# abhisrkckl/PulsePortraiture

Hardware: AMD Instinct MI355X
Metric: subint portrait fits/sec (phase+DM, 512ch×2048bin) at 1/2/4/8 MI355X (higher is better)
Workload: dtype f64

## Files before the change

pulseportraiture_amd/csrc/ppf_api.cpp:

```cpp
#include <hip/hip_runtime.h>

#include <algorithm>
#include <atomic>
#include <chrono>
#include <cmath>
#include <cstdarg>
#include <cstdio>
#include <cstdlib>
#include <cstring>
#include <map>
#include <mutex>
#include <string>
#include <thread>
#include <utility>
#include <vector>

#include "../../include/ppfit.h"
#include "ppf_internal.hpp"
#include "ppf_device.hpp"

struct ppf_ctx {
    int device;
    std::string err;
    mutable std::mutex err_mu;
// ... 337 lines not shown
    if (!d) return fail(ctx, PPF_EINVAL, "null descriptor");
    if (d->nsub < 1 || d->nchan < 1) return fail(ctx, PPF_EINVAL, "nsub=%d nchan=%d", d->nsub, d->nchan);
    if (!nbin_supported(d->nbin) && !long_fit_ok(d))
        return fail(ctx, PPF_EUNSUP,
                    "nbin=%d: must be even in [32, 8192] or odd in [33, 4095], or longer without the "
                    "GetTOAs guess (up to 2^23 transform points)", d->nbin);
    if (d->data_dtype != PPF_F32 && d->data_dtype != PPF_F64)
        return fail(ctx, PPF_EINVAL, "data_dtype=%d", d->data_dtype);
    if (d->nmodel < 1) return fail(ctx, PPF_EINVAL, "nmodel=%d", d->nmodel);
    if (!d->data || !d->model || !d->freqs || !d->P || !d->init || !d->fit_flags || !d->nu_fits ||
        !d->nu_outs || !d->results || !d->scales || !d->scale_errs || !d->channel_snrs ||
        !d->covariance)
        return fail(ctx, PPF_EINVAL, "required pointer is NULL");
    if (d->mode != PPF_MODE_FULL && d->mode != PPF_MODE_LEGACY2)
        return fail(ctx, PPF_EINVAL, "mode=%d", d->mode);
    if (d->guess) {
        if (!d->guess_weights || !d->guess_DM) return fail(ctx, PPF_EINVAL, "guess needs weights and DM");
        if (d->guess_Ns < 1 || d->guess_Ns > 65536) return fail(ctx, PPF_EINVAL, "guess_Ns=%d", d->guess_Ns);
    }
    if (!d->workspace) return fail(ctx, PPF_EINVAL, "workspace is NULL");
    FitLayout L = fit_layout(d);
    if (d->workspace_bytes < L.total)
        return fail(ctx, PPF_ENOMEM, "workspace %zu < %zu bytes", d->workspace_bytes, L.total);
    return PPF_OK;
}

using EvPair = std::pair<hipEvent_t, hipEvent_t>;

EvPair *event_pair(std::vector<EvPair> &v, int i, hipError_t *e) {
    if ((int)v.size() <= i) {
        EvPair pr{};
        if ((*e = hipEventCreate(&pr.first)) != hipSuccess) return nullptr;
        if ((*e = hipEventCreate(&pr.second)) != hipSuccess) {
            (void)hipEventDestroy(pr.first);
            return nullptr;
        }
        v.push_back(pr);
    }
    return &v[i];
}

int event_ms(ppf_ctx *ctx, hipEvent_t a, hipEvent_t b, double *ms) {
    hipError_t e = hipEventSynchronize(b);
    if (e != hipSuccess) return hip_fail(ctx, e, "hipEventSynchronize");
    float t = 0.f;
    if ((e = hipEventElapsedTime(&t, a, b)) != hipSuccess) return hip_fail(ctx, e, "hipEventElapsedTime");
    *ms = (double)t;
    return PPF_OK;
}

template <class F>
int for_history(ppf_ctx *ctx, int n, const double *ms, F &&entry) {
    if (!ctx || !ms || n < 0) return PPF_EINVAL;
    if (!ctx->prof) return fail(ctx, PPF_EINVAL, "profiling is off");
    const long avail = ctx->ncalls < ppf_ctx::kRing ? ctx->ncalls : ppf_ctx::kRing;
    if (n > avail) n = (int)avail;
    for (int c = 0; c < n; ++c)
        if (int rc = entry(c, (int)((ctx->ncalls - n + c) % ppf_ctx::kRing))) return rc;
    return n;
}

struct FitCall {
    ppf_ctx *ctx;
    const ppf_fit_desc *d;
    hipStream_t st;
    FitLayout L;
    char *ws;
    const double2 *T, *T2;
    double2 *Mft;
    double *Mpow;
    int nharm, kc;
    int slot;
    bool fused;
    bool bounded;
    uint8_t *needx;
    int32_t *xslot;
    uint8_t *xtile;
    uint8_t *gflag;
    double2 *gpart;
    double *gwx;
    unsigned *kinds;
    int32_t *cls;
    double *rec;

    template <class U>
    U *at(size_t off) const { return (U *)(ws + off); }
    const int32_t *KC() const { return at<const int32_t>(L.KC); }
    unsigned *counts() const { return kinds + 4; }
    void mark(int i) const { if (ctx->prof) (void)hipEventRecord(ctx->ring[slot][i], st); }
    EvPair *solv_begin(int kind) const {
        hipError_t e;
        EvPair *pe = ctx->prof ? event_pair(ctx->solv_ev[slot], ctx->nsolv[slot], &e) : nullptr;
        if (!pe) return nullptr;
        ctx->solv_kind[slot].resize(ctx->solv_ev[slot].size());
        ctx->solv_kind[slot][ctx->nsolv[slot]++] = kind;
        (void)hipEventRecord(pe->first, st);
        return pe;
    }
    void solv_end(EvPair *pe) const { if (pe) (void)hipEventRecord(pe->second, st); }

    int begin();
    int models(), spectra(), guess();
    ppf::SolveArgs solve_args() const;
    ppf::XmomArgs xmom_args(const ppf::SolveArgs &sa) const;
    int round(const ppf::SolveArgs &sa, const ppf::XmomArgs &ma, bool any_pass, bool any_mom, bool first);
    int solve(const ppf::SolveArgs &sa), postfit(const ppf::SolveArgs &sa);
};

int FitCall::begin() {
    hipError_t e = hipSetDevice(ctx->device);
    if (e != hipSuccess) return hip_fail(ctx, e, "hipSetDevice");
    L = fit_layout(d);
    int rc;
    if (!L.lng && (rc = twiddles(ctx, d->nbin, st, &T, &T2))) return rc;
    ws = (char *)d->workspace;
    Mft = at<double2>(L.M); Mpow = at<double>(L.Mpow);
    nharm = d->nbin / 2 + 1; kc = noise_kc(nharm, 4);
    fused = L.fused && !L.momx;
    bounded = (d->options & PPF_OPT_NO_X) != 0;
    needx = at<uint8_t>(L.needx); xslot = at<int32_t>(L.xslot);
    xtile = L.tiled ? at<uint8_t>(L.xtile) : nullptr;
    if (d->guess && L.fused && ppf::xspec_guess_fused_n(rfft_log2(d->nbin))) {
        gflag = at<uint8_t>(L.gflag); gpart = at<double2>(L.gpart); gwx = at<double>(L.gwx);
    }
    kinds = at<unsigned>(L.active + 16); cls = at<int32_t>(L.cls); rec = at<double>(L.rec);
    slot = (int)(ctx->ncalls % ppf_ctx::kRing);
    for (int i = 0; i < 4; ++i) ctx->ran[slot][i] = true;
    ctx->npass[slot] = ctx->nsolv[slot] = 0;
    ctx->ran[slot][2] = d->guess != 0;
    ctx->ran[slot][4] = ctx->ran[slot][5] = false;
    return PPF_OK;
}

int FitCall::models() {
    hipError_t e;
    if (L.lng) {
        if (int rc = long_rfft_rows(ctx, L.lw, ws, d->nbin, (int64_t)d->nmodel * d->nchan, PPF_F64, d->model, Mft,
                                    false, st))
            return rc;
    } else {
        ppf::RfftArgs ra{d->nbin, rfft_log2(d->nbin), PPF_F64, d->model, T, T2, Mft};
        if ((e = ppf::launch_rfft_rows(ra, (int64_t)d->nmodel * d->nchan, st)) != hipSuccess)
            return hip_fail(ctx, e, "k_rfft_rows");
    }
    if ((e = ppf::launch_model_pow_t(Mft, d->nchan, nharm, d->nmodel, at<double>(L.MP), st)) != hipSuccess)
        return hip_fail(ctx, e, "k_model_pow_t");
    if ((e = ppf::launch_model_cut(at<const double>(L.MP), d->nchan, nharm, d->nmodel,
                                   (d->options & PPF_OPT_NO_HCUT) != 0, at<int32_t>(L.KC), st)) != hipSuccess)
        return hip_fail(ctx, e, "k_model_cut");
    if ((e = ppf::launch_model_pow(Mft, d->nchan, nharm, d->nmodel, Mpow, st)) != hipSuccess)
        return hip_fail(ctx, e, "k_model_pow");
    if ((e = hipMemsetAsync(kinds, 0, 8 * sizeof(unsigned), st)) != hipSuccess)
        return hip_fail(ctx, e, "hipMemsetAsync");
    ppf::ClassifyArgs ca{};
    ca.nsub = d->nsub; ca.nchan = d->nchan; ca.log10_tau = d->log10_tau;
    ca.fused = fused ? 1 : 0; ca.xcap = L.xcap;
    ca.fit_flags = d->fit_flags; ca.init = d->init; ca.freqs = d->freqs; ca.P = d->P;
    ca.nu_fits = d->nu_fits; ca.mask = d->chan_mask; ca.model_index = d->model_index;
    ca.KC = KC(); ca.klim = gflag ? 64 * ppf::guess_npl(rfft_log2(d->nbin)) : -1;
    ca.guess_DM = d->guess ? d->guess_DM : nullptr; ca.guess_ref = d->guess ? d->guess_ref : 0;
    ca.needx = needx; ca.xslot = xslot; ca.xtile = xtile; ca.gflag = gflag; ca.cls = cls; ca.rec = rec;
    ca.hm_list = at<int32_t>(L.hmlist); ca.ng_list = at<int32_t>(L.nglist); ca.counts = counts();
    if ((e = ppf::launch_classify(ca, st)) != hipSuccess) return hip_fail(ctx, e, "k_classify");
    return PPF_OK;
}

// ... 124 lines not shown
    if (mr.cb > 8) {
        mr.cb = 8;
        mr.nblk = (mr.nchan + 7) / 8;
        mr.xcd_swizzle = (mr.nblk % 8 == 0) ? 1 : 0;
    }
    return mr;
}

int FitCall::round(const ppf::SolveArgs &sa, const ppf::XmomArgs &ma, bool any_pass, bool any_mom, bool first) {
    hipError_t e;
    if (any_pass) {
        EvPair *pe = nullptr;
        if (ctx->prof) {
            if (!(pe = event_pair(ctx->pass_ev[slot], ctx->npass[slot], &e)))
                return hip_fail(ctx, e, "hipEventCreate");
            ++ctx->npass[slot];
            (void)hipEventRecord(pe->first, st);
        }
        if ((e = ppf::launch_pass(sa, st)) != hipSuccess) return hip_fail(ctx, e, "k_pass");
        if (pe) (void)hipEventRecord(pe->second, st);
    }
    if (any_mom) {
        if (first) mark(5);
        if (!fused) e = ppf::launch_moments(sa, st);
        else e = first ? ppf::launch_xmom(ma, true, st) : ppf::launch_xmom(recentre_args(ma), false, st);
        if (e != hipSuccess) return hip_fail(ctx, e, fused ? "k_xmom" : "k_moments");
        if (first) {
            mark(6);
            ctx->ran[slot][4] = true;
        }
    }
    if ((e = hipMemsetAsync(sa.active, 0, 2 * sizeof(unsigned), st)) != hipSuccess)
        return hip_fail(ctx, e, "hipMemsetAsync");
    if (any_pass) {
        EvPair *pe = solv_begin(1);
        if ((e = ppf::launch_tr_step(sa, st)) != hipSuccess) return hip_fail(ctx, e, "k_tr_step");
        solv_end(pe);
    }
    if (any_mom) {
        EvPair *pe = solv_begin(0);
        if ((e = ppf::launch_tr_mom(sa, st)) != hipSuccess) return hip_fail(ctx, e, "k_tr_mom");
        solv_end(pe);
    }
    return PPF_OK;
}

int FitCall::solve(const ppf::SolveArgs &sa) {
    hipError_t e;
    int rc;
    if (!ctx->host_active && (e = hipHostMalloc((void **)&ctx->host_active, 4 * sizeof(unsigned))) != hipSuccess)
        return hip_fail(ctx, e, "hipHostMalloc");
    if ((e = ppf::launch_tr_init(sa, st)) != hipSuccess) return hip_fail(ctx, e, "k_tr_init");
    const bool spin = (d->options & PPF_OPT_SPIN_WAIT) != 0;
    const bool no_stream = L.fused && L.xcap == 0;
    bool kinds_late = !no_stream && bounded;
    bool any_mom = true, any_pass = false;
    if (!no_stream && !kinds_late) {
        if ((rc = read_back(ctx, ctx->host_active + 1, sa.kinds, 2, st, spin))) return rc;
        any_mom = ctx->host_active[1] != 0;
        any_pass = ctx->host_active[2] != 0;
    }
    const ppf::XmomArgs ma = xmom_args(sa);
    if (fused && (e = ppf::launch_btab(d->nbin / 2, at<double>(L.Bt), st)) != hipSuccess)
        return hip_fail(ctx, e, "k_btab");
    const int maxiter = d->max_iter > 0 ? d->max_iter : 200 * 5;
    int iter = 0;
    for (int group = any_pass ? 3 : 1; any_mom || any_pass; group = 2) {
        for (int g = 0; g < group; ++g)
            if ((rc = round(sa, ma, any_pass, any_mom, iter == 0 && g == 0))) return rc;
        iter += group;
        if (kinds_late && (e = hipMemcpyAsync(ctx->host_active + 1, sa.kinds, 2 * sizeof(unsigned),
                                              hipMemcpyDeviceToHost, st)) != hipSuccess)
            return hip_fail(ctx, e, "hipMemcpyAsync");
        if ((rc = read_back(ctx, ctx->host_active, sa.active, 1, st, spin))) return rc;
        if (kinds_late) {
            kinds_late = false;
            if (ctx->host_active[2] != 0) {
                any_pass = true;
                continue;
            }
        }
        if (*ctx->host_active == 0 || iter > maxiter + 2) break;
    }
    return PPF_OK;
}

int FitCall::postfit(const ppf::SolveArgs &sa) {
    EvPair *pe = solv_begin(2);
    const hipError_t e = ppf::launch_postfit(sa, st);
    if (e != hipSuccess) return hip_fail(ctx, e, "k_postfit");
    solv_end(pe);
    return PPF_OK;
}

}

extern "C" {

int ppf_abi_version(void) { return PPF_ABI_VERSION; }
size_t ppf_sizeof_fit_desc(void) { return sizeof(ppf_fit_desc); }
size_t ppf_sizeof_result(void) { return sizeof(ppf_result); }

int ppf_create(int device, ppf_ctx **out) {
    if (!out) return PPF_EINVAL;
    *out = nullptr;
    int n = 0;
    hipError_t e = hipGetDeviceCount(&n);
    if (e != hipSuccess || n == 0) return PPF_EHIP;
    if (device < 0 || device >= n) return PPF_EINVAL;
    ppf_ctx *c = new ppf_ctx();
    c->device = device;
    *out = c;
    return PPF_OK;
}

void ppf_destroy(ppf_ctx *ctx) {
    if (!ctx) return;
    (void)hipSetDevice(ctx->device);
    for (auto &kv : ctx->tw) (void)hipFree(kv.second);
    for (auto &kv : ctx->cz) (void)hipFree(kv.second);
    for (auto &set : ctx->ring)
        for (auto &e : set)
            if (e) (void)hipEventDestroy(e);
    for (auto &v : ctx->pass_ev)
        for (auto &pr : v) {
            (void)hipEventDestroy(pr.first);
            (void)hipEventDestroy(pr.second);
        }
    for (auto &v : ctx->solv_ev)
        for (auto &pr : v) {
            (void)hipEventDestroy(pr.first);
            (void)hipEventDestroy(pr.second);
        }
    if (ctx->host_active) (void)hipHostFree(ctx->host_active);
    if (ctx->lscr) (void)hipFree(ctx->lscr);
    delete ctx;
}

int ppf_set_profiling(ppf_ctx *ctx, int enable) {
    if (!ctx) return PPF_EINVAL;
    hipError_t e = hipSetDevice(ctx->device);
    if (e != hipSuccess) return hip_fail(ctx, e, "hipSetDevice");
    if (enable && !ctx->ring[0][0])
        for (auto &set : ctx->ring)
            for (auto &ev : set)
                if ((e = hipEventCreate(&ev)) != hipSuccess) return hip_fail(ctx, e, "hipEventCreate");
    ctx->prof = enable != 0;
    ctx->ncalls = 0;
    return PPF_OK;
}

int ppf_stage_ms_history(ppf_ctx *ctx, int n, double *ms) {
    return for_history(ctx, n, ms, [&](int c, int slot) -> int {
        for (int i = 0; i < 4; ++i) {
            ms[c * 4 + i] = 0.0;
            if (!ctx->ran[slot][i]) continue;
            if (int rc = event_ms(ctx, ctx->ring[slot][i], ctx->ring[slot][i + 1], &ms[c * 4 + i])) return rc;
        }
        return PPF_OK;
    });
}

int ppf_kernel_ms_history(ppf_ctx *ctx, int n, double *ms) {
    return for_history(ctx, n, ms, [&](int c, int slot) -> int {
        for (int i = 0; i < 2; ++i) {
            ms[c * 2 + i] = 0.0;
            if (!ctx->ran[slot][4 + i]) continue;
            if (int rc = event_ms(ctx, ctx->ring[slot][5 + 2 * i], ctx->ring[slot][6 + 2 * i], &ms[c * 2 + i]))
                return rc;
        }
        return PPF_OK;
    });
// ... 1251 lines not shown
```

pulseportraiture_amd/csrc/ppf_internal.hpp:

```cpp
#pragma once
#include <hip/hip_runtime.h>
#include <stdint.h>

#include "../../include/ppfit.h"

namespace ppf {

struct RfftArgs {
    int nbin, log2N, dtype;
    const void *in;
    const double2 *T, *T2;
    double2 *out;
};

struct XspecArgs {
    int nsub, nchan, nbin, log2N, kc, nblk, cb, dtype, xcd_swizzle;
    const void *data;
    const double2 *Mft;
    const int32_t *model_index;
    const uint8_t *mask;
    const double *errs;
    const double *freqs, *P;
    const double2 *T, *T2;
    double2 *X;
// ... 42 lines not shown
    const void *data;
    const double2 *Mft;
    const int32_t *model_index;
    const uint8_t *mask;
    double *chan;
    const double *dphi;
    const double2 *T, *T2;
    const void *state;
    double *mom;
    const double *Bt;
    int kc;
    const double *errs;
    const double *Mpow;
    double *mres;
    const int32_t *KC;
    const unsigned *rc_count;
    const int32_t *rc_list;
};

struct GuessArgs {
    int nsub, nchan, nbin, log2N, kc, nblkd, Ns;
    int guess_ref;
    const uint8_t *mask;
    const double *freqs, *P, *guess_DM, *guess_tau, *nu_fits;
    const double *gP;
    const double *gw;
    const double2 *T, *T2;
    double *x0;
    const double2 *Msum;
    const double2 *Mft;
    const int32_t *model_index;
    const int32_t *KC;
    const uint8_t *gflag;
    const double2 *gpart;
    const double *gwx;
    int nblk;
    const double2 *czB, *czT;
    int czP, czJ, czQ, czK;
    const double2 *gspec;
    double *gsh;
};

struct CzPlan {
    int Ns, K, P, J, Q;
};
hipError_t launch_cz_table(const CzPlan &c, double2 *B, const double2 *T, hipStream_t st);

struct TRState;

struct SolveArgs {
    int nsub, nchan, nbin;
    const double2 *X, *Mft;
    const double *MP;
    const int32_t *KC;
    const int32_t *model_index;
    const double *chan;
    const double *freqs, *P;
    const uint8_t *mask;
    const double *init;
    const int32_t *fit_flags;
    const double *nu_fits, *nu_outs;
    const double *bounds;
    int log10_tau, option, is_toa, mode, max_iter, guess;
    int newton;
    const double *x0;
    double *stats;
    ppf_result *results;
    double *scales, *scale_errs, *channel_snrs, *covariance;
    TRState *state;
    double *partials;
    unsigned *active;
    unsigned *kinds;
    double2 *mom;
    double *dphi;
    double *mres;
    int mom16;
    double *hcen;
    const int32_t *xslot;
    const uint8_t *xtile;
    int xnh;
    unsigned *rc_count;
    int32_t *rc_list;
    const double *rec;
};

struct RotateArgs {
    int nbin, log2N, dtype;
    const void *in;
    const double *phases;
    const double2 *T, *T2;
    double *out;
    int ref_len;
    const double2 *Te, *T2e;
};

struct InstRespArgs {
    int nbin;
    const double *src;
    const int32_t *src_row;
    const double *table;
    const double *widths;
    const double2 *T, *T2;
    double *out;
};

struct AlignArgs {
    int nsub, nchan, nbin, log2N, dtype, ngroup;
    const void *in;
    const double *phases;
    const double *weights;
    const double2 *T, *T2;
    double2 *part;
    double *wpart;
    double *out;
    double *wsum;
};
int align_groups(int nsub, int nchan);
hipError_t launch_align(const AlignArgs &a, hipStream_t st);
bool align_wave_supported(int log2N);
hipError_t launch_align_part_w(const AlignArgs &a, hipStream_t st);
hipError_t launch_align_phases(int nsub, int nchan, const double *results, const double *freqs, const double *P,
                               const uint8_t *mask, const double *scales, const double *errs, double *phases,
                               double *weights, hipStream_t st);

struct ResidArgs {
    int nbin, log2N, dtype;
    const void *in;
    const double *phases;
    const double *model;
    const int32_t *model_row;
    const double *scales, *errs;
    double dof;
    const double2 *T, *T2;
    double *out;
};
hipError_t launch_resid_chi2(const ResidArgs &a, int64_t nrows, hipStream_t st);

struct NoiseArgs {
    int nbin, log2N, dtype, kc;
    const void *in;
    const double2 *T, *T2;
    double *out;
};

constexpr int kNfGrid = 20;
struct NoiseFitArgs {
    int nbin, dtype;
    const void *in;
    const double2 *T, *T2;
    int64_t nharm;
    const double *pows;
    const double *errs;
    int64_t errs_len;
    int fn;
    double fact;
    double a_grid[kNfGrid];
    int32_t kc_table[kNfGrid];
    double *noise_out;
    int32_t *kc_out;
    int64_t row0;
};

struct LongNoiseArgs {
    int64_t nbin;
    int64_t n;
    int64_t M, M1, M2;
    int log2M, log2M1;
// ... 303 lines not shown
```

pulseportraiture_amd/csrc/ppf_solve.hip:

```cpp
#include <type_traits>
#include "ppf_device.hpp"
#include "ppf_internal.hpp"
#include "ppf_state.hpp"

namespace ppf {

struct Fac {
    double dphi[3];
    double t[2];
    double u[3];
    bool br_tt, br_ta, br_aa;
};

__device__ __forceinline__ void chan_derivs(const double *st, const Fac &fc, double dC[5],
                                            double dS[5], double d2C[5][5], double d2S[5][5]) {
    const double Cp = st[1], Cpp = st[2], Q1 = st[3], Q1p = st[4], Q2 = st[5];
    const double S1 = st[7], S2a = st[8], S2b = st[9];
    for (int i = 0; i < 3; ++i) { dC[i] = Cp * fc.dphi[i]; dS[i] = 0.0; }
    for (int j = 0; j < 2; ++j) { dC[3 + j] = Q1 * fc.t[j]; dS[3 + j] = S1 * fc.t[j]; }
    for (int i = 0; i < 3; ++i) {
        for (int j = 0; j < 3; ++j) { d2C[i][j] = Cpp * fc.dphi[i] * fc.dphi[j]; d2S[i][j] = 0.0; }
        for (int j = 0; j < 2; ++j) {
            d2C[i][3 + j] = d2C[3 + j][i] = fc.dphi[i] * fc.t[j] * Q1p;
            d2S[i][3 + j] = d2S[3 + j][i] = 0.0;
// ... 1232 lines not shown
                double co[7] = {A * C - E * G, 0.0, E * H - A * D, 0.0, F * G - B * C, 0.0,
                                B * D - F * H};
                double roots[8];
                int nr = poly_real_roots(co, 6, roots);
                double best = 0.0, bd = 1e300;
                bool any = false;
                for (int i = 0; i < nr; ++i)
                    if (roots[i] > 0.0 && fabs(nu_mean - roots[i]) < bd) {
                        bd = fabs(nu_mean - roots[i]); best = roots[i]; any = true;
                    }
                if (any) { nz[0] = nz[1] = best; } else no_root = true;
            }
            break;
        }
        case 0x1b: {
            double T[4][4];
            int q = 12;
            for (int i = 0; i < 4; ++i)
                for (int j = i; j < 4; ++j) { T[i][j] = T[j][i] = c[q]; ++q; }
            double H11 = T[0][0], H22 = T[1][1], H33 = T[2][2], H44 = T[3][3];
            double H12 = T[0][1], H13 = T[0][2], H14 = T[0][3], H23 = T[1][2],
                   H34 = T[2][3];
            num = (H34 * H34 - H33 * H44) * c[0] + (H13 * H44 - H14 * H34) * c[1] +
                  (H14 * H33 - H13 * H34) * c[2];
            den = (H34 * H34 - H33 * H44) * c[3] + (H13 * H44 - H14 * H34) * c[4] +
                  (H14 * H33 - H13 * H34) * c[5];
            nz[0] = pow(num / den, -0.5);
            num = (H13 * H22 - H12 * H23) * c[6] + (H11 * H23 - H12 * H13) * c[7] +
                  (H12 * H12 - H11 * H22) * c[8];
            den = (H13 * H22 - H12 * H23) * c[9] + (H11 * H23 - H12 * H13) * c[10] +
                  (H12 * H12 - H11 * H22) * c[11];
            nz[2] = exp(num / den);
            break;
        }
        case 0xf: {
            if (option == 0 || option == 1) {
                double H14 = c[16], H44 = c[17];
                double A = c[0], aa = c[1], B = c[2], b = c[3], C = c[4], cc = c[5],
                       D = c[6], d = c[7], E = c[8], e = c[9], F = c[10], f = c[11];
                double co[6];
                int deg;
                if (option == 0) {
                    co[0] = A * A * B + H44 * C * D + H14 * E * F - H44 * B * E - A * C * F -
                            H14 * A * D;
                    co[1] = -A * A * b - H44 * C * d - H14 * E * f + H44 * b * E + A * C * f +
                            H14 * A * d;
                    co[2] = -2 * A * aa * B - H44 * cc * D - H14 * e * F + H44 * B * e +
                            (A * cc + aa * C) * F + H14 * aa * D;
                    co[3] = 2 * A * aa * b + H44 * cc * d + H14 * e * f - H44 * b * e -
                            (A * cc + aa * C) * f - H14 * aa * d;
                    co[4] = aa * aa * B - aa * cc * F;
                    co[5] = -aa * aa * b + aa * cc * f;
                    deg = 5;
                } else {
                    co[0] = A * A * B + H44 * C * D + H14 * E * F - H44 * B * E - A * C * F -
                            H14 * A * D;
                    co[1] = -2 * A * aa * B - H44 * cc * D - H14 * e * F + H44 * B * e +
                            (A * cc + aa * C) * F + H14 * aa * D;
                    co[2] = -(A * A * b - aa * aa * B) - H44 * C * d - H14 * E * f +
                            H44 * b * E + (A * C * f - aa * cc * F) + H14 * A * d;
                    co[3] = 2 * A * aa * b + H44 * cc * d + H14 * e * f - H44 * b * e -
                            (A * cc + aa * C) * f - H14 * aa * d;
                    co[4] = -aa * aa * b + aa * cc * f;
                    deg = 4;
                }
                double roots[8];
                int nr = poly_real_roots(co, deg, roots);
                double best = 0.0, bd = 1e300;
                bool any = false;
                for (int i = 0; i < nr; ++i)
                    if (roots[i] > 0.0) {
                        double rr = sqrt(roots[i]);
                        if (fabs(nu_mean - rr) < bd) { bd = fabs(nu_mean - rr); best = rr; any = true; }
                    }
                if (any) { nz[0] = nz[1] = best; } else no_root = true;
            }
            break;
        }
        default: break;
    }
    *no_root_out = no_root ? 1 : 0;
}

template <int PB>
__global__ __launch_bounds__(PB) void k_postfit(SolveArgs a) {
    __shared__ double red[kWaves * 32];
    __shared__ double sh_Xinv[25];
    __shared__ double sh_misc[16];
    __shared__ double sh_acc[NZ_MAX + 8];
    const int s = blockIdx.x, tid = threadIdx.x;
    const TRState &S = a.state[s];
    ppf_result *res = a.results + s;
    if (S.status == PPF_ST_NOFIT || S.status == PPF_ST_NOSPACE) {
        if (tid == 0) {
            for (int i = 0; i < 32; ++i) reinterpret_cast<double *>(res)[i] = 0.0;
            res->status = S.status;
            const double pg = S.phi_guess;
            res->phi_guess = fabs(pg) <= kDblMax ? pg : a.init[(int64_t)s * 5];
        }
        for (int n = tid; n < a.nchan; n += PB) {
            const int64_t o2 = (int64_t)s * a.nchan + n;
            a.scales[o2] = 0.0; a.scale_errs[o2] = 0.0; a.channel_snrs[o2] = 0.0;
        }
        return;
    }
    struct { const double *fr; const uint8_t *mask; int nchan; } v;
    v.fr = a.freqs + (int64_t)s * a.nchan;
    v.mask = a.mask ? a.mask + (int64_t)s * a.nchan : nullptr;
    v.nchan = a.nchan;
    const int flagmask = S.flagmask;
    int idx[5], nf = 0;
    for (int i = 0; i < 5; ++i)
        if (flagmask >> i & 1) idx[nf++] = i;
    double x[5];
    for (int i = 0; i < 5; ++i) x[i] = S.x[i];
    const double fun = S.f;
    const int status = S.status, nfev = S.nfev, k = S.k;
    const bool scat = S.scat != 0;
    const double nu_mean = S.nu_mean, dof = S.dof, phi_guess = S.phi_guess;
    double sdv[1] = {0.0};
    {
        const double *chan = a.chan + (int64_t)s * a.nchan * 4;
        const uint8_t *mk = a.mask ? a.mask + (int64_t)s * a.nchan : nullptr;
        for (int n = tid; n < a.nchan; n += PB)
            if (!mk || mk[n]) sdv[0] += chan[n * 4 + 2];
    }
    blk_sum<1, PB>(sdv, red);
    const double Sd = sdv[0];
    const int nchanx = S.nchanx;
    FitGeom g;
    g.P = a.P[s];
    g.nu_DM = S.nu_fit[0];
    g.nu_GM = S.nu_fit[1];
    g.nu_tau = S.nu_fit[2];
    g.log10_tau = a.log10_tau;
    g.tau_lin = 0.0;
    g.g_sum = g.g_tau = g.g_alpha = false;
    const double *st_fit = a.stats + ((int64_t)s * 2 + S.slot_cur) * a.nchan * 10;

    const double tau_fit_lin = a.log10_tau ? pow(10.0, x[3]) : x[3];
    auto gates = [&](FitGeom &gg, double taulin, double alpha) {
        gg.tau_lin = taulin;
        if (!scat) { gg.g_sum = gg.g_tau = gg.g_alpha = false; return; }
        double sm[3] = {0.0, 0.0, 0.0};
        for (int n = tid; n < v.nchan; n += PB) {
            if (v.mask && !v.mask[n]) continue;
            double tn = taulin * pow(v.fr[n] / gg.nu_tau, alpha);
            sm[0] += tn;
            sm[1] += gg.log10_tau ? kLn10 * tn : tn / taulin;
            sm[2] += log(v.fr[n] / gg.nu_tau) * tn;
        }
        blk_sum<3, PB>(sm, red);
        gg.g_sum = sm[0] != 0.0;
        gg.g_tau = gg.g_sum && sm[1] != 0.0;
        gg.g_alpha = sm[2] != 0.0;
    };
    gates(g, tau_fit_lin, x[4]);

    double nu_out[3];
    bool need_nz = false;
    for (int i = 0; i < 3; ++i) {
        nu_out[i] = a.nu_outs[(int64_t)s * 3 + i];
        if (!(nu_out[i] == nu_out[i]) || nu_out[i] == 0.0) need_nz = true;
    }
    int nzcase = flagmask;
    if (a.mode == PPF_MODE_LEGACY2) nzcase = 0x3;
    if (nzcase == 0x1f) nzcase = 0x1b;
    double nz[3] = {g.nu_DM, g.nu_GM, g.nu_tau};
    bool no_root = false;
    const bool closed = (nzcase == 0x3 || nzcase == 0x5 || nzcase == 0x18 || nzcase == 0xb ||
                         nzcase == 0x7 || nzcase == 0x1b || nzcase == 0xf);
    if (need_nz && closed) {
        double accv[NZ_MAX + 8];
        for (int i = 0; i < NZ_MAX + 8; ++i) accv[i] = 0.0;
        const double cD = kDconst / g.P, cG = kDconst * kDconst / g.P;
        for (int n = tid; n < v.nchan; n += PB) {
            if (v.mask && !v.mask[n]) continue;
            const double *st = st_fit + (int64_t)n * 10;
            const double nu = v.fr[n];
            Fac fc = make_fac(nu, g, x[4]);
            double H[5][5], Hd[5][5], Hg[5][5], Ha[5][5];
            chan_hess(st, fc, H);
            Fac f1 = fc; f1.dphi[1] = 1.0; chan_hess(st, f1, Hd);
            Fac f2 = fc; f2.dphi[2] = 1.0; chan_hess(st, f2, Hg);
            double rd[5], rg[5], ra[5];
            for (int b = 0; b < 5; ++b) { rd[b] = Hd[1][b]; rg[b] = Hg[2][b]; }
            rd[1] = Hd[1][1] * fc.dphi[1];
            rg[2] = Hg[2][2] * fc.dphi[2];
            if (nzcase == 0x18 || nzcase == 0x1b) {
                Fac f3 = fc;
                if (fc.t[1] != 0.0) {
                    f3.u[1] = fc.u[1] / fc.t[1];
                    f3.u[2] = fc.u[2] / fc.t[1];
                }
                f3.t[1] = 1.0;
                chan_hess(st, f3, Ha);
                for (int b = 0; b < 5; ++b) ra[b] = Ha[4][b];
            }
            const double w2 = pow(nu, -2.0), w4 = pow(nu, -4.0), wl = log(nu);
            double *c = accv;
            switch (nzcase) {
                case 0x3: c[0] += w2 * rd[0]; c[1] += rd[0]; break;
                case 0x5: c[0] += w4 * rg[0]; c[1] += rg[0]; break;
                case 0x18: c[0] += wl * ra[3]; c[1] += ra[3]; break;
                case 0xb:
                    c[0] += w2 * rd[3]; c[1] += w2 * rd[0]; c[2] += rd[3]; c[3] += rd[0];
                    c[16] += H[3][0]; c[17] += H[3][3];
                    break;
                case 0x7:
                    if (a.option == 0) {
                        c[0] += w4 * rg[0]; c[1] += rg[0]; c[2] += w2 * rd[2]; c[3] += rd[2];
                        c[4] += w4 * rg[2]; c[5] += rg[2]; c[6] += w2 * rd[0]; c[7] += rd[0];
                    } else {
                        c[0] += w4 * rd[0]; c[1] += rd[0]; c[2] += w2 * rg[1]; c[3] += rg[1];
                        c[4] += w4 * rd[1]; c[5] += rd[1]; c[6] += w2 * rg[0]; c[7] += rg[0];
                    }
                    break;
                case 0x1b:
                    c[0] += w2 * rd[0]; c[1] += w2 * rd[3]; c[2] += w2 * rd[4];
                    c[3] += rd[0]; c[4] += rd[3]; c[5] += rd[4];
                    c[6] += wl * ra[0]; c[7] += wl * ra[1]; c[8] += wl * ra[3];
                    c[9] += ra[0]; c[10] += ra[1]; c[11] += ra[3];
                    {
                        const int r4[4] = {0, 1, 3, 4};
                        int q = 12;
                        for (int i = 0; i < 4; ++i)
                            for (int j = i; j < 4; ++j) c[q++] += H[r4[i]][r4[j]];
                    }
                    break;
                case 0xf: {
                    double d0 = rd[0] * cD, d1 = rd[1] * cD, d2 = rd[2] * cD, d3 = rd[3] * cD;
                    double e0 = rg[0] * cG, e1 = rg[1] * cG, e2 = rg[2] * cG, e3 = rg[3] * cG;
                    if (a.option == 0) {
                        c[0] += w4 * e3; c[1] += e3; c[2] += w2 * d0; c[3] += d0;
                        c[4] += w4 * e0; c[5] += e0; c[6] += w2 * d2; c[7] += d2;
                        c[8] += w4 * e2; c[9] += e2; c[10] += w2 * d3; c[11] += d3;
                    } else {
                        c[0] += w2 * d3; c[1] += d3; c[2] += w4 * e0; c[3] += e0;
                        c[4] += w2 * d0; c[5] += d0; c[6] += w4 * e1; c[7] += e1;
                        c[8] += w2 * d1; c[9] += d1; c[10] += w4 * e3; c[11] += e3;
                    }
                    c[16] += H[3][0]; c[17] += H[3][3];
                    break;
                }
                default: break;
            }
        }
        blk_sum<NZ_MAX + 8, PB>(accv, red);
        if (tid == 0) {
            for (int i = 0; i < NZ_MAX + 8; ++i) sh_acc[i] = accv[i];
            int nr_flag = 0;
            nz_solve(sh_acc, nzcase, a.option, nu_mean, nz, &nr_flag);
            no_root = nr_flag != 0;
            sh_misc[4] = nz[0]; sh_misc[5] = nz[1]; sh_misc[6] = nz[2];
            sh_misc[7] = no_root ? 1.0 : 0.0;
        }
        __syncthreads();
        nz[0] = sh_misc[4]; nz[1] = sh_misc[5]; nz[2] = sh_misc[6];
        no_root = sh_misc[7] != 0.0;
        __syncthreads();
    }
    if (need_nz)
        for (int i = 0; i < 3; ++i)
            if (!(nu_out[i] == nu_out[i]) || nu_out[i] == 0.0) nu_out[i] = nz[i];
    if (a.mode == PPF_MODE_LEGACY2) { nu_out[1] = nu_out[0]; nu_out[2] = g.nu_tau; }
    if (a.is_toa) {
        if (flagmask & 2) nu_out[1] = nu_out[0];
        else if (flagmask & 4) nu_out[0] = nu_out[1];
    }

    const double P = g.P;
    double phi_inf = x[0] + kDconst * x[1] * (0.0 - pow(g.nu_DM, -2.0)) / P +
                     kDconst * kDconst * x[2] * (0.0 - pow(g.nu_GM, -4.0)) / P;
    double phi_out = phi_inf + (kDconst / P) * x[1] * pow(nu_out[0], -2.0) +
                     (kDconst * kDconst / P) * x[2] * pow(nu_out[1], -4.0);
    if (fabs(phi_out) >= 0.5) phi_out = phi_out - floor(phi_out);
    if (phi_out >= 0.5) phi_out -= 1.0;
    double tau_out_lin = tau_fit_lin * pow(nu_out[2] / g.nu_tau, x[4]);
    double tau_out = a.log10_tau ? log10(tau_out_lin) : tau_out_lin;

    FitGeom go = g;
    go.nu_DM = nu_out[0];
    go.nu_GM = nu_out[1];
    go.nu_tau = nu_out[2];
    gates(go, tau_out_lin, x[4]);
    double cv[31];
    for (int i = 0; i < 31; ++i) cv[i] = 0.0;
    for (int n = tid; n < v.nchan; n += PB) {
        if (v.mask && !v.mask[n]) continue;
        const double *st = st_fit + (int64_t)n * 10;
        Fac fc = make_fac(v.fr[n], go, x[4]);
        double dC[5], dS[5], d2C[5][5], d2S[5][5];
        chan_derivs(st, fc, dC, dS, d2C, d2S);
        const double C = st[0], S = st[6], an = C / S;
        double U[5];
        for (int i = 0; i < 5; ++i) U[i] = (flagmask >> i & 1) ? -2.0 * (dC[i] - an * dS[i]) : 0.0;
        const double cinv = 1.0 / (2.0 * S);
        int q = 0;
        for (int i = 0; i < 5; ++i)
            for (int j = i; j < 5; ++j) {
                if ((flagmask >> i & 1) && (flagmask >> j & 1)) {
                    cv[q] += -2.0 * (C * d2C[i][j] / S - 0.5 * C * C * d2S[i][j] / (S * S));
                    cv[15 + q] += U[i] * U[j] * cinv;
                }
                ++q;
            }
    }
    blk_sum<31, PB>(cv, red);
    int sing = 0;
    if (tid == 0) {
        double Xm[5][5], Xi[5][5];
        double full[5][5];
        int q = 0;
        for (int i = 0; i < 5; ++i)
            for (int j = i; j < 5; ++j) { full[i][j] = full[j][i] = cv[q] - cv[15 + q]; ++q; }
        for (int i2 = 0; i2 < nf; ++i2)
            for (int j2 = 0; j2 < nf; ++j2) Xm[i2][j2] = full[idx[i2]][idx[j2]];
        if (!invert_small(Xm, Xi, nf)) sing = 1;
        for (int i2 = 0; i2 < 25; ++i2) sh_Xinv[i2] = 0.0;
        for (int i2 = 0; i2 < nf; ++i2)
            for (int j2 = 0; j2 < nf; ++j2) sh_Xinv[idx[i2] * 5 + idx[j2]] = Xi[i2][j2];
        sh_misc[8] = (double)sing;
    }
    __syncthreads();
    sing = (int)sh_misc[8];
    double Xinv[5][5];
    for (int i2 = 0; i2 < 5; ++i2)
        for (int j2 = 0; j2 < 5; ++j2) Xinv[i2][j2] = sh_Xinv[i2 * 5 + j2];
    double sn[1] = {0.0};
    for (int n = tid; n < v.nchan; n += PB) {
        const int64_t o2 = (int64_t)s * a.nchan + n;
        if (v.mask && !v.mask[n]) {
            a.scales[o2] = 0.0; a.scale_errs[o2] = 0.0; a.channel_snrs[o2] = 0.0;
            continue;
        }
        const double *st = st_fit + (int64_t)n * 10;
        Fac fc = make_fac(v.fr[n], go, x[4]);
        double dC[5], dS[5], d2C[5][5], d2S[5][5];
        chan_derivs(st, fc, dC, dS, d2C, d2S);
        const double C = st[0], S = st[6], an = C / S;
        double U[5];
#pragma unroll
        for (int i2 = 0; i2 < 5; ++i2) U[i2] = (flagmask >> i2 & 1) ? -2.0 * (dC[i2] - an * dS[i2]) : 0.0;
        double quad = 0.0;
#pragma unroll
        for (int i2 = 0; i2 < 5; ++i2)
#pragma unroll
            for (int j2 = 0; j2 < 5; ++j2)
                if ((flagmask >> i2 & 1) && (flagmask >> j2 & 1)) quad += U[i2] * Xinv[i2][j2] * U[j2];
        const double cinv = 1.0 / (2.0 * S);
        double var = 2.0 * (cinv + quad * cinv * cinv);
        double serr = (a.mode == PPF_MODE_LEGACY2) ? pow(S, -0.5) : sqrt(var);
        double csnr = an * sqrt(S);
        a.scales[o2] = an;
        a.scale_errs[o2] = serr;
        a.channel_snrs[o2] = csnr;
        sn[0] += csnr * csnr;
    }
    blk_sum<1, PB>(sn, red);
    if (tid == 0) {
        double pe[5] = {0, 0, 0, 0, 0};
        double *cov = a.covariance + (int64_t)s * 25;
        for (int i2 = 0; i2 < 25; ++i2) cov[i2] = 0.0;
        for (int i2 = 0; i2 < nf; ++i2) {
            for (int j2 = 0; j2 < nf; ++j2) cov[i2 * 5 + j2] = 2.0 * sh_Xinv[idx[i2] * 5 + idx[j2]];
            pe[idx[i2]] = sqrt(2.0 * sh_Xinv[idx[i2] * 5 + idx[i2]]);
        }
        double params[5] = {phi_out, x[1], x[2], tau_out, x[4]};
        for (int i2 = 0; i2 < 5; ++i2) { res->params[i2] = params[i2]; res->param_errs[i2] = pe[i2]; }
        for (int i2 = 0; i2 < 3; ++i2) res->nu_out[i2] = nu_out[i2];
        res->nu_fit[0] = g.nu_DM; res->nu_fit[1] = g.nu_GM; res->nu_fit[2] = g.nu_tau;
        res->chi2 = Sd + fun;
        res->red_chi2 = (Sd + fun) / dof;
        res->snr = sqrt(sn[0]);
        res->fun = fun;
        res->Sd = Sd;
        res->phi_guess = phi_guess;
        res->nfeval = (double)nfev;
        int st2 = status;
        if (no_root) st2 |= PPF_ST_NO_ROOT;
        if (sing) st2 |= PPF_ST_SINGULAR;
        if (!(fun == fun)) st2 |= PPF_ST_NONFINITE;
        res->status = (double)st2;
        res->niter = (double)k;
        res->dof = dof;
        res->nchanx = (double)nchanx;
        res->x_fit_phi = x[0];
        res->x_fit_tau = x[3];
        double npass = S.mmode ? (double)S.nmom + 1.0 : (double)nfev;
        if (!S.mmode && S.nsubev > 0) {
            const int ng = (a.nchan + 63) / 64, nsel = (ng + S.sub0 - 1) / S.sub0;
            npass -= (double)S.nsubev * (1.0 - (double)nsel / (double)ng);
        }
        res->npass = npass;
        res->reserved[0] = res->reserved[1] = 0.0;
    }
}

hipError_t launch_classify(const ClassifyArgs &a, hipStream_t st) {
    constexpr int NW = kClassifyBlock / 64;
    hipLaunchKernelGGL(k_classify, dim3((unsigned)((a.nsub + NW - 1) / NW)), dim3(kClassifyBlock), 0, st, a);
    return hipGetLastError();
}

hipError_t launch_tr_init(const SolveArgs &a, hipStream_t st) {
    hipLaunchKernelGGL(k_tr_init, dim3((unsigned)((a.nsub + kWaves - 1) / kWaves)), dim3(kBlock), 0,
                       st, a);
    return hipGetLastError();
}

hipError_t launch_pass(const SolveArgs &a, hipStream_t st) {
    const int nblk = (a.nchan + kPassChans - 1) / kPassChans;
    hipLaunchKernelGGL(k_pass, dim3((unsigned)((int64_t)a.nsub * nblk)), dim3(kBlock), 0, st, a);
    return hipGetLastError();
}

hipError_t launch_tr_step(const SolveArgs &a, hipStream_t st) {
    const dim3 g((unsigned)((a.nsub + kWaves - 1) / kWaves));
    const bool lane = a.nsub >= 2048 && a.nchan <= 2048;
    if (lane) {
        const dim3 gl((unsigned)((a.nsub + 63) / 64));
        const size_t lds = 64 * sizeof(TRState);
        if (a.bounds) hipLaunchKernelGGL(k_tr_step_l<true>, gl, dim3(64), lds, st, a);
        else hipLaunchKernelGGL(k_tr_step_l<false>, gl, dim3(64), lds, st, a);
        hipError_t e = hipGetLastError();
        if (e != hipSuccess) return e;
        hipLaunchKernelGGL(k_tr_gates, g, dim3(kBlock), 0, st, a);
        return hipGetLastError();
    }
    if (a.bounds)
        hipLaunchKernelGGL(k_tr_step<true>, g, dim3(kBlock), 0, st, a);
    else
        hipLaunchKernelGGL(k_tr_step<false>, g, dim3(kBlock), 0, st, a);
    return hipGetLastError();
}

hipError_t launch_moments(const SolveArgs &a, hipStream_t st) {
    const int nblk = (a.nchan + kMomChans - 1) / kMomChans;
    if (a.mom16) hipLaunchKernelGGL(k_moments<true>, dim3((unsigned)((int64_t)a.nsub * nblk)), dim3(kBlock), 0, st, a);
    else hipLaunchKernelGGL(k_moments<false>, dim3((unsigned)((int64_t)a.nsub * nblk)), dim3(kBlock), 0, st, a);
    return hipGetLastError();
}

hipError_t launch_tr_mom(const SolveArgs &a, hipStream_t st) {
    hipLaunchKernelGGL(k_tr_mom<128>, dim3((unsigned)a.nsub), dim3(128), 0, st, a);
    return hipGetLastError();
}

hipError_t launch_postfit(const SolveArgs &a, hipStream_t st) {
    const int pb = a.nchan <= 2048 ? 64 : 256;
    if (pb == 64) hipLaunchKernelGGL(k_postfit<64>, dim3((unsigned)a.nsub), dim3(64), 0, st, a);
    else hipLaunchKernelGGL(k_postfit<256>, dim3((unsigned)a.nsub), dim3(256), 0, st, a);
    return hipGetLastError();
}

size_t tr_state_bytes() { return sizeof(TRState); }
int pass_blocks(int nchan) { return (nchan + kPassChans - 1) / kPassChans; }

}

#ifdef PPF_TM_PROF
extern "C" int ppf_debug_tprof(unsigned long long *out, int reset) {
    if (hipMemcpyFromSymbol(out, HIP_SYMBOL(ppf::g_tprof), sizeof(unsigned long long) * 8) != hipSuccess)
        return -1;
    if (reset) {
        unsigned long long z[8] = {};
        if (hipMemcpyToSymbol(HIP_SYMBOL(ppf::g_tprof), z, sizeof(z)) != hipSuccess) return -1;
    }
    return 0;
}
#endif
```

Before: 372,700.

## Add specialized postfit kernel for non-scattering subints and skip unneeded launches

Adds k_postfit_mom, a slimmed postfit kernel for subints without scattering. It uses a 3x3 phase/DM Hessian, smaller reductions, and a shared-memory table of per-channel frequency powers when the block is 64 threads. The host tracks whether any pass or moment-mode subints ran and sets pf_skip so each postfit kernel launches only when needed. The generic kernel now returns early for subints the specialized kernel handles. This adds a second code path that must match the original numerics, plus optional profiling macros.

```diff
diff --git a/pulseportraiture_amd/csrc/ppf_api.cpp b/pulseportraiture_amd/csrc/ppf_api.cpp
--- a/pulseportraiture_amd/csrc/ppf_api.cpp
+++ b/pulseportraiture_amd/csrc/ppf_api.cpp
@@ -443,6 +443,7 @@
     unsigned *kinds;
     int32_t *cls;
     double *rec;
+    int pf_skip;
 
     template <class U>
     U *at(size_t off) const { return (U *)(ws + off); }
@@ -733,12 +734,15 @@
         }
         if (*ctx->host_active == 0 || iter > maxiter + 2) break;
     }
+    pf_skip = !any_pass ? ppf::kPfSkipFull : (!any_mom ? ppf::kPfSkipMom : 0);
     return PPF_OK;
 }
 
 int FitCall::postfit(const ppf::SolveArgs &sa) {
     EvPair *pe = solv_begin(2);
-    const hipError_t e = ppf::launch_postfit(sa, st);
+    ppf::SolveArgs pa = sa;
+    pa.pf_skip = pf_skip;
+    const hipError_t e = ppf::launch_postfit(pa, st);
     if (e != hipSuccess) return hip_fail(ctx, e, "k_postfit");
     solv_end(pe);
     return PPF_OK;
diff --git a/pulseportraiture_amd/csrc/ppf_internal.hpp b/pulseportraiture_amd/csrc/ppf_internal.hpp
--- a/pulseportraiture_amd/csrc/ppf_internal.hpp
+++ b/pulseportraiture_amd/csrc/ppf_internal.hpp
@@ -148,7 +148,9 @@
     unsigned *rc_count;
     int32_t *rc_list;
     const double *rec;
-};
+    int pf_skip;
+};
+enum { kPfSkipMom = 1, kPfSkipFull = 2 };
 
 struct RotateArgs {
     int nbin, log2N, dtype;
diff --git a/pulseportraiture_amd/csrc/ppf_solve.hip b/pulseportraiture_amd/csrc/ppf_solve.hip
--- a/pulseportraiture_amd/csrc/ppf_solve.hip
+++ b/pulseportraiture_amd/csrc/ppf_solve.hip
@@ -1338,6 +1338,78 @@
     *no_root_out = no_root ? 1 : 0;
 }
 
+#ifdef PPF_PF_PROF
+__device__ unsigned long long g_pfprof[8];
+#define PF_INIT() unsigned long long pf_acc[8] = {0, 0, 0, 0, 0, 0, 0, 0}; unsigned long long pf_t = __builtin_amdgcn_s_memtime()
+#define PF(i) do { const unsigned long long pf_n = __builtin_amdgcn_s_memtime(); pf_acc[i] += pf_n - pf_t; pf_t = pf_n; } while (0)
+#define PF_DONE() do { if (tid == 0) for (int ti = 0; ti < 8; ++ti) atomicAdd(&g_pfprof[ti], pf_acc[ti]); } while (0)
+#else
+#define PF_INIT()
+#define PF(i)
+#define PF_DONE()
+#endif
+template <int PB>
+__device__ __forceinline__ void postfit_nofit(const SolveArgs &a, int s, const TRState &S) {
+    const int tid = threadIdx.x;
+    ppf_result *res = a.results + s;
+    if (tid == 0) {
+        for (int i = 0; i < 32; ++i) reinterpret_cast<double *>(res)[i] = 0.0;
+        res->status = S.status;
+        const double pg = S.phi_guess;
+        res->phi_guess = fabs(pg) <= kDblMax ? pg : a.init[(int64_t)s * 5];
+    }
+    for (int n = tid; n < a.nchan; n += PB) {
+        const int64_t o2 = (int64_t)s * a.nchan + n;
+        a.scales[o2] = 0.0; a.scale_errs[o2] = 0.0; a.channel_snrs[o2] = 0.0;
+    }
+}
+
+struct PostfitOut {
+    double phi_out, tau_out, Sd, fun, dof, phi_guess, snr2;
+    double x[5], nu_out[3], nu_fit[3];
+    int status, nfev, k, nchanx, nf, idx[5];
+    bool no_root, sing;
+};
+
+__device__ __forceinline__ void postfit_record(const SolveArgs &a, int s, const TRState &S,
+                                               const PostfitOut &o, const double *Xinv) {
+    ppf_result *res = a.results + s;
+    double pe[5] = {0, 0, 0, 0, 0};
+    double *cov = a.covariance + (int64_t)s * 25;
+    for (int i2 = 0; i2 < 25; ++i2) cov[i2] = 0.0;
+    for (int i2 = 0; i2 < o.nf; ++i2) {
+        for (int j2 = 0; j2 < o.nf; ++j2) cov[i2 * 5 + j2] = 2.0 * Xinv[o.idx[i2] * 5 + o.idx[j2]];
+        pe[o.idx[i2]] = sqrt(2.0 * Xinv[o.idx[i2] * 5 + o.idx[i2]]);
+    }
+    double params[5] = {o.phi_out, o.x[1], o.x[2], o.tau_out, o.x[4]};
+    for (int i2 = 0; i2 < 5; ++i2) { res->params[i2] = params[i2]; res->param_errs[i2] = pe[i2]; }
+    for (int i2 = 0; i2 < 3; ++i2) { res->nu_out[i2] = o.nu_out[i2]; res->nu_fit[i2] = o.nu_fit[i2]; }
+    res->chi2 = o.Sd + o.fun;
+    res->red_chi2 = (o.Sd + o.fun) / o.dof;
+    res->snr = sqrt(o.snr2);
+    res->fun = o.fun;
+    res->Sd = o.Sd;
+    res->phi_guess = o.phi_guess;
+    res->nfeval = (double)o.nfev;
+    int st2 = o.status;
+    if (o.no_root) st2 |= PPF_ST_NO_ROOT;
+    if (o.sing) st2 |= PPF_ST_SINGULAR;
+    if (!(o.fun == o.fun)) st2 |= PPF_ST_NONFINITE;
+    res->status = (double)st2;
+    res->niter = (double)o.k;
+    res->dof = o.dof;
+    res->nchanx = (double)o.nchanx;
+    res->x_fit_phi = o.x[0];
+    res->x_fit_tau = o.x[3];
+    double npass = S.mmode ? (double)S.nmom + 1.0 : (double)o.nfev;
+    if (!S.mmode && S.nsubev > 0) {
+        const int ng = (a.nchan + 63) / 64, nsel = (ng + S.sub0 - 1) / S.sub0;
+        npass -= (double)S.nsubev * (1.0 - (double)nsel / (double)ng);
+    }
+    res->npass = npass;
+    res->reserved[0] = res->reserved[1] = 0.0;
+}
+
 template <int PB>
 __global__ __launch_bounds__(PB) void k_postfit(SolveArgs a) {
     __shared__ double red[kWaves * 32];
@@ -1346,18 +1418,10 @@
     __shared__ double sh_acc[NZ_MAX + 8];
     const int s = blockIdx.x, tid = threadIdx.x;
     const TRState &S = a.state[s];
-    ppf_result *res = a.results + s;
-    if (S.status == PPF_ST_NOFIT || S.status == PPF_ST_NOSPACE) {
-        if (tid == 0) {
-            for (int i = 0; i < 32; ++i) reinterpret_cast<double *>(res)[i] = 0.0;
-            res->status = S.status;
-            const double pg = S.phi_guess;
-            res->phi_guess = fabs(pg) <= kDblMax ? pg : a.init[(int64_t)s * 5];
-        }
-        for (int n = tid; n < a.nchan; n += PB) {
-            const int64_t o2 = (int64_t)s * a.nchan + n;
-            a.scales[o2] = 0.0; a.scale_errs[o2] = 0.0; a.channel_snrs[o2] = 0.0;
-        }
+    const bool unfit = S.status == PPF_ST_NOFIT || S.status == PPF_ST_NOSPACE;
+    if (!(a.pf_skip & kPfSkipMom) && (unfit || !S.scat)) return;
+    if (unfit) {
+        postfit_nofit<PB>(a, s, S);
         return;
     }
     struct { const double *fr; const uint8_t *mask; int nchan; } v;
@@ -1374,6 +1438,7 @@
     const int status = S.status, nfev = S.nfev, k = S.k;
     const bool scat = S.scat != 0;
     const double nu_mean = S.nu_mean, dof = S.dof, phi_guess = S.phi_guess;
+    PF_INIT();
     double sdv[1] = {0.0};
     {
         const double *chan = a.chan + (int64_t)s * a.nchan * 4;
@@ -1412,6 +1477,7 @@
         gg.g_alpha = sm[2] != 0.0;
     };
     gates(g, tau_fit_lin, x[4]);
+    PF(0);
 
     double nu_out[3];
     bool need_nz = false;
@@ -1503,6 +1569,7 @@
             }
         }
         blk_sum<NZ_MAX + 8, PB>(accv, red);
+        PF(1);
         if (tid == 0) {
             for (int i = 0; i < NZ_MAX + 8; ++i) sh_acc[i] = accv[i];
             int nr_flag = 0;
@@ -1515,6 +1582,7 @@
         nz[0] = sh_misc[4]; nz[1] = sh_misc[5]; nz[2] = sh_misc[6];
         no_root = sh_misc[7] != 0.0;
         __syncthreads();
+        PF(2);
     }
     if (need_nz)
         for (int i = 0; i < 3; ++i)
@@ -1563,6 +1631,7 @@
             }
     }
     blk_sum<31, PB>(cv, red);
+    PF(3);
     int sing = 0;
     if (tid == 0) {
         double Xm[5][5], Xi[5][5];
@@ -1580,6 +1649,7 @@
     }
     __syncthreads();
     sing = (int)sh_misc[8];
+    PF(4);
     double Xinv[5][5];
     for (int i2 = 0; i2 < 5; ++i2)
         for (int j2 = 0; j2 < 5; ++j2) Xinv[i2][j2] = sh_Xinv[i2 * 5 + j2];
@@ -1614,7 +1684,9 @@
         sn[0] += csnr * csnr;
     }
     blk_sum<1, PB>(sn, red);
+    PF(5);
     if (tid == 0) {
+        ppf_result *res = a.results + s;
         double pe[5] = {0, 0, 0, 0, 0};
         double *cov = a.covariance + (int64_t)s * 25;
         for (int i2 = 0; i2 < 25; ++i2) cov[i2] = 0.0;
@@ -1651,6 +1723,252 @@
         res->npass = npass;
         res->reserved[0] = res->reserved[1] = 0.0;
     }
+    PF(6);
+    PF_DONE();
+}
+
+__device__ __noinline__ double2 pf_powers(double nu, bool want2, bool want4) {
+    double2 w;
+    w.x = want2 ? pow(nu, -2.0) : 0.0;
+    w.y = want4 ? pow(nu, -4.0) : 0.0;
+    return w;
+}
+
+__device__ __forceinline__ double mom_hess(double C, double iS, double d2c, double dci, double dcj) {
+    return -2.0 * fma(dci * dcj, iS, C * d2c * iS);
+}
+
+__device__ __noinline__ bool pf_invert(double (*Xm)[5], double (*Xi)[5], int nf) {
+    return invert_small(Xm, Xi, nf);
+}
+
+template <int PB>
+__global__ __launch_bounds__(PB) void k_postfit_mom(SolveArgs a) {
+    constexpr bool tab = PB == 64;
+    extern __shared__ double sh_pw[];
+    __shared__ double red[kWaves * 12];
+    __shared__ double sh_Xinv[25];
+    __shared__ double sh_misc[16];
+    __shared__ double sh_acc[8];
+    const int s = blockIdx.x, tid = threadIdx.x;
+    const TRState &S = a.state[s];
+    const bool unfit = S.status == PPF_ST_NOFIT || S.status == PPF_ST_NOSPACE;
+    if (!unfit && S.scat) return;
+    if (unfit) {
+        postfit_nofit<PB>(a, s, S);
+        return;
+    }
+    const int nchan = a.nchan;
+    const double *fr = a.freqs + (int64_t)s * nchan;
+    const uint8_t *mask = a.mask ? a.mask + (int64_t)s * nchan : nullptr;
+    const int flagmask = S.flagmask & 0x7;
+    int idx[5] = {0, 0, 0, 0, 0}, nf = 0;
+    for (int i = 0; i < 3; ++i)
+        if (flagmask >> i & 1) idx[nf++] = i;
+    double x[5];
+    for (int i = 0; i < 5; ++i) x[i] = S.x[i];
+    const double fun = S.f;
+    const int status = S.status, nfev = S.nfev, k = S.k;
+    const double nu_mean = S.nu_mean, dof = S.dof, phi_guess = S.phi_guess;
+    PF_INIT();
+    double sdv[1] = {0.0};
+    {
+        const double *chan = a.chan + (int64_t)s * nchan * 4;
+        for (int n = tid; n < nchan; n += PB)
+            if (!mask || mask[n]) sdv[0] += chan[n * 4 + 2];
+    }
+    blk_sum<1, PB>(sdv, red);
+    const double Sd = sdv[0];
+    const int nchanx = S.nchanx;
+    const double P = a.P[s];
+    const double nu_fit[3] = {S.nu_fit[0], S.nu_fit[1], S.nu_fit[2]};
+    const double *st_fit = a.stats + ((int64_t)s * 2 + S.slot_cur) * nchan * 10;
+    const double tau_fit_lin = a.log10_tau ? pow(10.0, x[3]) : x[3];
+
+    double nu_out[3];
+    bool need_nz = false;
+    for (int i = 0; i < 3; ++i) {
+        nu_out[i] = a.nu_outs[(int64_t)s * 3 + i];
+        if (!(nu_out[i] == nu_out[i]) || nu_out[i] == 0.0) need_nz = true;
+    }
+    int nzcase = flagmask;
+    if (a.mode == PPF_MODE_LEGACY2) nzcase = 0x3;
+    const bool closed = nzcase == 0x3 || nzcase == 0x5 || nzcase == 0x7;
+    const bool nz_run = need_nz && closed;
+    const bool want2 = (flagmask & 2) || (nz_run && nzcase == 0x3);
+    const bool want4 = (flagmask & 4) != 0;
+    if constexpr (tab)
+        for (int n = tid; n < nchan; n += PB) {
+            if (mask && !mask[n]) continue;
+            const double2 w = pf_powers(fr[n], want2, want4);
+            sh_pw[n] = w.x;
+            sh_pw[nchan + n] = w.y;
+        }
+    auto powers = [&](int n) {
+        if constexpr (tab) return make_double2(sh_pw[n], sh_pw[nchan + n]);
+        else return pf_powers(fr[n], want2, want4);
+    };
+    PF(0);
+
+    double nz[3] = {nu_fit[0], nu_fit[1], nu_fit[2]};
+    bool no_root = false;
+    if (nz_run) {
+        double accv[8];
+        for (int i = 0; i < 8; ++i) accv[i] = 0.0;
+        const double rDM = pow(nu_fit[0], -2.0), rGM = pow(nu_fit[1], -4.0);
+        for (int n = tid; n < nchan; n += PB) {
+            if (mask && !mask[n]) continue;
+            const double *st = st_fit + (int64_t)n * 10;
+            const double C = st[0], Cp = st[1], Cpp = st[2], iS = 1.0 / st[6];
+            const double2 w = powers(n);
+            const double w2 = w.x, w4 = w.y;
+            const double h0 = mom_hess(C, iS, Cpp, Cp, Cp);
+            double *c = accv;
+            switch (nzcase) {
+                case 0x3: c[0] += w2 * h0; c[1] += h0; break;
+                case 0x5: c[0] += w4 * h0; c[1] += h0; break;
+                case 0x7:
+                    if (a.option == 0) {
+                        const double dphi2 = kDconst * kDconst * (w4 - rGM) / P;
+                        const double rd2 = mom_hess(C, iS, Cpp * dphi2, Cp, Cp * dphi2);
+                        const double rg2 = h0 * dphi2;
+                        c[0] += w4 * h0; c[1] += h0; c[2] += w2 * rd2; c[3] += rd2;
+                        c[4] += w4 * rg2; c[5] += rg2; c[6] += w2 * h0; c[7] += h0;
+                    } else {
+                        const double dphi1 = kDconst * (w2 - rDM) / P;
+                        const double rg1 = mom_hess(C, iS, Cpp * dphi1, Cp, Cp * dphi1);
+                        const double rd1 = h0 * dphi1;
+                        c[0] += w4 * h0; c[1] += h0; c[2] += w2 * rg1; c[3] += rg1;
+                        c[4] += w4 * rd1; c[5] += rd1; c[6] += w2 * h0; c[7] += h0;
+                    }
+                    break;
+                default: break;
+            }
+        }
+        blk_sum<8, PB>(accv, red);
+        PF(1);
+        if (tid == 0) {
+            for (int i = 0; i < 8; ++i) sh_acc[i] = accv[i];
+            int nr_flag = 0;
+            nz_solve(sh_acc, nzcase, a.option, nu_mean, nz, &nr_flag);
+            sh_misc[4] = nz[0]; sh_misc[5] = nz[1]; sh_misc[6] = nz[2];
+            sh_misc[7] = nr_flag ? 1.0 : 0.0;
+        }
+        __syncthreads();
+        nz[0] = sh_misc[4]; nz[1] = sh_misc[5]; nz[2] = sh_misc[6];
+        no_root = sh_misc[7] != 0.0;
+        __syncthreads();
+        PF(2);
+    }
+    if (need_nz)
+        for (int i = 0; i < 3; ++i)
+            if (!(nu_out[i] == nu_out[i]) || nu_out[i] == 0.0) nu_out[i] = nz[i];
+    if (a.mode == PPF_MODE_LEGACY2) { nu_out[1] = nu_out[0]; nu_out[2] = nu_fit[2]; }
+    if (a.is_toa) {
+        if (flagmask & 2) nu_out[1] = nu_out[0];
+        else if (flagmask & 4) nu_out[0] = nu_out[1];
+    }
+
+    double phi_inf = x[0] + kDconst * x[1] * (0.0 - pow(nu_fit[0], -2.0)) / P +
+                     kDconst * kDconst * x[2] * (0.0 - pow(nu_fit[1], -4.0)) / P;
+    double phi_out = phi_inf + (kDconst / P) * x[1] * pow(nu_out[0], -2.0) +
+                     (kDconst * kDconst / P) * x[2] * pow(nu_out[1], -4.0);
+    if (fabs(phi_out) >= 0.5) phi_out = phi_out - floor(phi_out);
+    if (phi_out >= 0.5) phi_out -= 1.0;
+    double tau_out_lin = tau_fit_lin * pow(nu_out[2] / nu_fit[2], x[4]);
+    double tau_out = a.log10_tau ? log10(tau_out_lin) : tau_out_lin;
+
+    const double oDM = pow(nu_out[0], -2.0), oGM = pow(nu_out[1], -4.0);
+    double cv[12];
+    for (int i = 0; i < 12; ++i) cv[i] = 0.0;
+    for (int n = tid; n < nchan; n += PB) {
+        if (mask && !mask[n]) continue;
+        const double *st = st_fit + (int64_t)n * 10;
+        const double C = st[0], Cp = st[1], Cpp = st[2], S6 = st[6];
+        const double2 w = powers(n);
+        const double dphi[3] = {1.0, kDconst * (w.x - oDM) / P, kDconst * kDconst * (w.y - oGM) / P};
+        double U[3];
+#pragma unroll
+        for (int i = 0; i < 3; ++i) U[i] = (flagmask >> i & 1) ? -2.0 * (Cp * dphi[i]) : 0.0;
+        const double cinv = 1.0 / (2.0 * S6);
+        int q = 0;
+#pragma unroll
+        for (int i = 0; i < 3; ++i)
+#pragma unroll
+            for (int j = i; j < 3; ++j) {
+                if ((flagmask >> i & 1) && (flagmask >> j & 1)) {
+                    cv[q] += -2.0 * (C * (Cpp * dphi[i] * dphi[j]) / S6);
+                    cv[6 + q] += U[i] * U[j] * cinv;
+                }
+                ++q;
+            }
+    }
+    blk_sum<12, PB>(cv, red);
+    PF(3);
+    int sing = 0;
+    if (tid == 0) {
+        double Xm[5][5], Xi[5][5];
+        double full[3][3];
+        int q = 0;
+        for (int i = 0; i < 3; ++i)
+            for (int j = i; j < 3; ++j) { full[i][j] = full[j][i] = cv[q] - cv[6 + q]; ++q; }
+        for (int i2 = 0; i2 < nf; ++i2)
+            for (int j2 = 0; j2 < nf; ++j2) Xm[i2][j2] = full[idx[i2]][idx[j2]];
+        if (!pf_invert(Xm, Xi, nf)) sing = 1;
+        for (int i2 = 0; i2 < 25; ++i2) sh_Xinv[i2] = 0.0;
+        for (int i2 = 0; i2 < nf; ++i2)
+            for (int j2 = 0; j2 < nf; ++j2) sh_Xinv[idx[i2] * 5 + idx[j2]] = Xi[i2][j2];
+        sh_misc[8] = (double)sing;
+    }
+    __syncthreads();
+    sing = (int)sh_misc[8];
+    PF(4);
+    double Xinv[3][3];
+    for (int i2 = 0; i2 < 3; ++i2)
+        for (int j2 = 0; j2 < 3; ++j2) Xinv[i2][j2] = sh_Xinv[i2 * 5 + j2];
+    double sn[1] = {0.0};
+    for (int n = tid; n < nchan; n += PB) {
+        const int64_t o2 = (int64_t)s * nchan + n;
+        if (mask && !mask[n]) {
+            a.scales[o2] = 0.0; a.scale_errs[o2] = 0.0; a.channel_snrs[o2] = 0.0;
+            continue;
+        }
+        const double *st = st_fit + (int64_t)n * 10;
+        const double C = st[0], Cp = st[1], S6 = st[6], an = C / S6;
+        const double2 w = powers(n);
+        const double dphi[3] = {1.0, kDconst * (w.x - oDM) / P, kDconst * kDconst * (w.y - oGM) / P};
+        double U[3];
+#pragma unroll
+        for (int i2 = 0; i2 < 3; ++i2) U[i2] = (flagmask >> i2 & 1) ? -2.0 * (Cp * dphi[i2]) : 0.0;
+        double quad = 0.0;
+#pragma unroll
+        for (int i2 = 0; i2 < 3; ++i2)
+#pragma unroll
+            for (int j2 = 0; j2 < 3; ++j2)
+                if ((flagmask >> i2 & 1) && (flagmask >> j2 & 1)) quad += U[i2] * Xinv[i2][j2] * U[j2];
+        const double cinv = 1.0 / (2.0 * S6);
+        double var = 2.0 * (cinv + quad * cinv * cinv);
+        double serr = (a.mode == PPF_MODE_LEGACY2) ? pow(S6, -0.5) : sqrt(var);
+        double csnr = an * sqrt(S6);
+        a.scales[o2] = an;
+        a.scale_errs[o2] = serr;
+        a.channel_snrs[o2] = csnr;
+        sn[0] += csnr * csnr;
+    }
+    blk_sum<1, PB>(sn, red);
+    PF(5);
+    if (tid == 0) {
+        PostfitOut o;
+        o.phi_out = phi_out; o.tau_out = tau_out; o.Sd = Sd; o.fun = fun; o.dof = dof;
+        o.phi_guess = phi_guess; o.snr2 = sn[0];
+        for (int i = 0; i < 5; ++i) { o.x[i] = x[i]; o.idx[i] = idx[i]; }
+        for (int i = 0; i < 3; ++i) { o.nu_out[i] = nu_out[i]; o.nu_fit[i] = nu_fit[i]; }
+        o.status = status; o.nfev = nfev; o.k = k; o.nchanx = nchanx; o.nf = nf;
+        o.no_root = no_root; o.sing = sing != 0;
+        postfit_record(a, s, S, o, sh_Xinv);
+    }
+    PF(6);
+    PF_DONE();
 }
 
 hipError_t launch_classify(const ClassifyArgs &a, hipStream_t st) {
@@ -1705,6 +2023,16 @@
 
 hipError_t launch_postfit(const SolveArgs &a, hipStream_t st) {
     const int pb = a.nchan <= 2048 ? 64 : 256;
+    if (!(a.pf_skip & kPfSkipMom)) {
+        if (pb == 64)
+            hipLaunchKernelGGL(k_postfit_mom<64>, dim3((unsigned)a.nsub), dim3(64),
+                               (size_t)a.nchan * 2 * sizeof(double), st, a);
+        else
+            hipLaunchKernelGGL(k_postfit_mom<256>, dim3((unsigned)a.nsub), dim3(256), 0, st, a);
+        const hipError_t e = hipGetLastError();
+        if (e != hipSuccess) return e;
+    }
+    if (a.pf_skip & kPfSkipFull) return hipSuccess;
     if (pb == 64) hipLaunchKernelGGL(k_postfit<64>, dim3((unsigned)a.nsub), dim3(64), 0, st, a);
     else hipLaunchKernelGGL(k_postfit<256>, dim3((unsigned)a.nsub), dim3(256), 0, st, a);
     return hipGetLastError();
@@ -1714,6 +2042,18 @@
 int pass_blocks(int nchan) { return (nchan + kPassChans - 1) / kPassChans; }
 
 }
+
+#ifdef PPF_PF_PROF
+extern "C" int ppf_debug_pfprof(unsigned long long *out, int reset) {
+    if (hipMemcpyFromSymbol(out, HIP_SYMBOL(ppf::g_pfprof), sizeof(unsigned long long) * 8) != hipSuccess)
+        return -1;
+    if (reset) {
+        unsigned long long z[8] = {};
+        if (hipMemcpyToSymbol(HIP_SYMBOL(ppf::g_pfprof), z, sizeof(z)) != hipSuccess) return -1;
+    }
+    return 0;
+}
+#endif
 
 #ifdef PPF_TM_PROF
 extern "C" int ppf_debug_tprof(unsigned long long *out, int reset) {
```

New measurement: 382,700, median of 6. 1.03x the previous value.
